# Animesh005/Torus-FHE

Measured on AMD Instinct MI355X. Metric: bootstrapped gates/sec (NAND, N=1024), higher is better.
Workload: dtype f64

## Files before the change

### torus-fhe_amd/csrc/thfhe_common.h

```cpp
#ifndef THFHE_COMMON_H
#define THFHE_COMMON_H

#include <hip/hip_runtime.h>

#include "../../include/thfhe_hip.h"
#include "thfhe_lane.h"

namespace thfhe {

constexpr int kOpIdentity = 100;

int thfhe_fail(int code, const char *msg);
int thfhe_fail_hip(hipError_t e, const char *what);

inline int ilog2(int x) {
    int l = 0;
    while ((1 << l) < x) l++;
    return l;
}

inline int lut_validate(const thfhe_lut_spec *sp, const void *tv, int n_luts, const int32_t *lut_index, const int32_t *in0, const int32_t *in1,
                        const int32_t *in2, const int32_t *out, size_t count, int max_luts = 1024) {
    if (!sp || !tv || !in0 || !out) return thfhe_fail(THFHE_E_INVALID, "null argument");
    if (sp->n_inputs < 1 || sp->n_inputs > 3) return thfhe_fail(THFHE_E_INVALID, "lut spec: n_inputs must be 1, 2 or 3");
// ... 76 lines not shown
    wave_sync();
    fwds_seg1(lane, z, xb, T1);
    wave_sync();
    fwds_seg2_ld(lane, z, xb);
    fwds_seg2_st(lane, z, xb, w);
    wave_sync();
    fwds_seg3(lane, z, xb);
}
__device__ __forceinline__ void wave_fft_inv_s(int lane, cplx (&z)[8], cplx *xb, const cplx *T1, const W64 &w) {
    wave_sync();
    invs_seg1(lane, z, xb, w);
    wave_sync();
    invs_seg2_ld(lane, z, xb);
    invs_seg2_st(lane, z, xb);
    wave_sync();
    invs_seg3(lane, z, xb, T1);
}
__device__ __forceinline__ void wave_fft_fwd_r(int lane, cplx (&z)[8], cplx *xb, const LaneRoots &r, const W64 &w) {
    wave_sync();
    fwdr_seg1(lane, z, xb, r);
    wave_sync();
    fwd_seg2_ld(lane, z, xb);
    fwdr_seg2_st(lane, z, xb, w);
    wave_sync();
    fwd_seg3(lane, z, xb);
}
__device__ __forceinline__ void wave_fft_inv_r(int lane, cplx (&z)[8], cplx *xb, const LaneRoots &r, const W64 &w) {
    wave_sync();
    invr_seg1(lane, z, xb, w);
    wave_sync();
    inv_seg2_ld(lane, z, xb);
    inv_seg2_st(lane, z, xb);
    wave_sync();
    invr_seg3(lane, z, xb, r);
}
__device__ __forceinline__ void wave_transpose_hi3(cplx (&z)[8]) {
    uint32_t w[8][4];
#pragma unroll
    for (int r = 0; r < 8; r++) __builtin_memcpy(w[r], &z[r], 16);
#pragma unroll
    for (int d = 0; d < 4; d++) {
#pragma unroll
        for (int r = 0; r < 4; r++) {
            auto q = __builtin_amdgcn_permlane32_swap(w[r][d], w[r + 4][d], false, false);
            w[r][d] = q[0];
            w[r + 4][d] = q[1];
        }
#pragma unroll
        for (int r = 0; r < 8; r++) {
            if (r & 2) continue;
            auto q = __builtin_amdgcn_permlane16_swap(w[r][d], w[r + 2][d], false, false);
            w[r][d] = q[0];
            w[r + 2][d] = q[1];
        }
#pragma unroll
        for (int r = 0; r < 8; r += 2) {
            const uint32_t a = w[r][d], b = w[r + 1][d];
            w[r + 1][d] = __builtin_amdgcn_update_dpp(b, a, 0x128, 0xF, 0x3, false);
            w[r][d] = __builtin_amdgcn_update_dpp(a, b, 0x128, 0xF, 0xC, false);
        }
    }
#pragma unroll
    for (int r = 0; r < 8; r++) __builtin_memcpy(&z[r], w[r], 16);
}
template <class Roots>
__device__ __forceinline__ void wave_fft_fwd_q(int lane, cplx (&z)[8], cplx *xb, const Roots &r, const W64 &w) {
    fwdq_seg1(z, r);
    wave_transpose_hi3(z);
    wave_sync();
    fwdr_seg2_st(lane, z, xb, w);
    wave_sync();
    fwd_seg3(lane, z, xb);
}
template <class Roots>
__device__ __forceinline__ void wave_fft_inv_q(int lane, cplx (&z)[8], cplx *xb, const Roots &r, const W64 &w) {
    wave_sync();
    invr_seg1(lane, z, xb, w);
    wave_sync();
    inv_seg2_ld(lane, z, xb);
    dft8<-1>(z);
    wave_transpose_hi3(z);
    invq_seg3(z, r);
}
template <class Roots>
__device__ __forceinline__ void wave_fft_fwd_qs(int lane, cplx (&z)[8], cplx *xb, const Roots &r, const W64 &w) {
    fwdq_seg1(z, r);
    wave_transpose_hi3(z);
    wave_sync();
    fwds_seg2_st(lane, z, xb, w);
    wave_sync();
    fwds_seg3(lane, z, xb);
}
template <class Roots>
__device__ __forceinline__ void wave_fft_inv_qs(int lane, cplx (&z)[8], cplx *xb, const Roots &r, const W64 &w) {
    wave_sync();
    invs_seg1(lane, z, xb, w);
    wave_sync();
    invs_seg2_ld(lane, z, xb);
    dft8<-1>(z);
    wave_transpose_hi3(z);
    invq_seg3(z, r);
}
template <int T>
__device__ __forceinline__ void wave_fft_fwd_t(int lane, cplx (&z)[8], cplx *xb, const cplx *T1t, const W64 &w) {
    wave_sync();
    fwdt_seg1<T>(lane, z, xb, T1t);
    wave_sync();
    fwds_seg2_ld(lane, z, xb);
    fwds_seg2_st(lane, z, xb, w);
    wave_sync();
    fwds_seg3(lane, z, xb);
}
template <int T>
__device__ __forceinline__ void wave_fft_inv_t(int lane, cplx (&z)[8], cplx *xb, const cplx *T1t, const W64 &w) {
    wave_sync();
    invs_seg1(lane, z, xb, w);
    wave_sync();
    invs_seg2_ld(lane, z, xb);
    invs_seg2_st(lane, z, xb);
    wave_sync();
    invt_seg3<T>(lane, z, xb, T1t);
}
template <int T, int DEN = 32>
__device__ __forceinline__ void wave_fft_fwd_tq(int lane, cplx (&z)[8], cplx *xb, const LaneRoots &r, const W64 &w) {
    fwdtq_seg1<T, DEN>(z, r);
    wave_transpose_hi3(z);
    wave_sync();
    fwds_seg2_st(lane, z, xb, w);
    wave_sync();
    fwds_seg3(lane, z, xb);
}
template <int T, int DEN = 32>
__device__ __forceinline__ void wave_fft_inv_tq(int lane, cplx (&z)[8], cplx *xb, const LaneRoots &r, const W64 &w) {
    wave_sync();
    invs_seg1(lane, z, xb, w);
    wave_sync();
    invs_seg2_ld(lane, z, xb);
    dft8<-1>(z);
    wave_transpose_hi3(z);
    invtq_seg3<T, DEN>(z, r);
}

template <int TA, int TB, int DEN = 32>
__device__ __forceinline__ void wave_fft_fwd_tq_two(int lane, cplx (&za)[8], cplx (&zb)[8], cplx *xa, cplx *xb, const LaneRoots &ra, const LaneRoots &rb,
                                                    const W64 &w) {
    fwdtq_seg1<TA, DEN>(za, ra);
    fwdtq_seg1<TB, DEN>(zb, rb);
    wave_transpose_hi3(za);
    wave_transpose_hi3(zb);
    wave_sync();
    fwds_seg2_st(lane, za, xa, w);
    fwds_seg2_st(lane, zb, xb, w);
    wave_sync();
    fwds_seg3(lane, za, xa);
    fwds_seg3(lane, zb, xb);
}
template <int TA, int TB, int DEN = 32>
__device__ __forceinline__ void wave_fft_inv_tq_two(int lane, cplx (&za)[8], cplx (&zb)[8], cplx *xb, const LaneRoots &ra, const LaneRoots &rb, const W64 &w) {
    wave_sync();
    invs_seg1(lane, za, xb, w);
    wave_sync();
    invs_seg2_ld(lane, za, xb);
    wave_sync();
    invs_seg1(lane, zb, xb, w);
    wave_sync();
    dft8<-1>(za);
// ... 13 lines not shown
```

### torus-fhe_amd/csrc/thfhe_lane.h

```cpp
#ifndef THFHE_LANE_H
#define THFHE_LANE_H

#include <limits.h>
#include <stddef.h>
#include <stdint.h>

#if defined(__HIPCC__)
#define THFHE_FN __host__ __device__ __forceinline__
#else
#define THFHE_FN inline __attribute__((always_inline))
#endif

namespace thfhe {

constexpr int kLanes = 64;
constexpr int kXbufSlots = 8 * 72;

struct alignas(16) cplx {
    double re, im;
};

THFHE_FN cplx cmul(cplx a, cplx b) { return cplx{a.re * b.re - a.im * b.im, a.re * b.im + a.im * b.re}; }
THFHE_FN cplx cmul_conj(cplx a, cplx b) {
    return cplx{a.re * b.re + a.im * b.im, a.im * b.re - a.re * b.im};
// ... 186 lines not shown
    dft8<+1>(z);
    cplx p[8];
    w64_powers(w, p);
    xbuf[xs_c(0, lane)] = z[0];
#pragma unroll
    for (int k1 = 1; k1 < 8; k1++) xbuf[xs_c(k1, lane)] = cmul(z[k1], p[k1]);
}
THFHE_FN void invr_seg1(int lane, cplx (&z)[8], cplx *xbuf, const W64 &w) {
    dft8<-1>(z);
    cplx p[8];
    w64_powers(w, p);
    xbuf[xs_d(0, lane)] = z[0];
#pragma unroll
    for (int j0 = 1; j0 < 8; j0++) xbuf[xs_d(j0, lane)] = cmul_conj(z[j0], p[j0]);
}
THFHE_FN void invr_seg3(int lane, cplx (&z)[8], const cplx *xbuf, const LaneRoots &r) {
    const cplx s2 = cmul(r.s, r.s);
    cplx e = r.b, o = cmul(r.b, r.s);
#pragma unroll
    for (int k0 = 0; k0 < 8; k0 += 2) {
        z[k0] = cmul_conj(xbuf[xs_a(k0, lane)], e);
        z[k0 + 1] = cmul_conj(xbuf[xs_a(k0 + 1, lane)], o);
        if (k0 < 6) {
            e = cmul(e, s2);
            o = cmul(o, s2);
        }
    }
    dft8<-1>(z);
#pragma unroll
    for (int m = 1; m < 8; m++) z[m] = cmul_conj(z[m], cplx{THFHE_C_RE(m), THFHE_C_IM(m)});
}

THFHE_FN void fwdq_seg1(cplx (&z)[8], const LaneRoots &r) {
#pragma unroll
    for (int m = 1; m < 8; m++) z[m] = cmul(z[m], cplx{THFHE_C_RE(m), THFHE_C_IM(m)});
    dft8<+1>(z);
    const cplx s2 = cmul(r.s, r.s);
    cplx e = r.b, o = cmul(r.b, r.s);
#pragma unroll
    for (int k0 = 0; k0 < 8; k0 += 2) {
        z[k0] = cmul(z[k0], e);
        z[k0 + 1] = cmul(z[k0 + 1], o);
        if (k0 < 6) {
            e = cmul(e, s2);
            o = cmul(o, s2);
        }
    }
}
THFHE_FN void invq_seg3(cplx (&z)[8], const LaneRoots &r) {
    const cplx s2 = cmul(r.s, r.s);
    cplx e = r.b, o = cmul(r.b, r.s);
#pragma unroll
    for (int k0 = 0; k0 < 8; k0 += 2) {
        z[k0] = cmul_conj(z[k0], e);
        z[k0 + 1] = cmul_conj(z[k0 + 1], o);
        if (k0 < 6) {
            e = cmul(e, s2);
            o = cmul(o, s2);
        }
    }
    dft8<-1>(z);
#pragma unroll
    for (int m = 1; m < 8; m++) z[m] = cmul_conj(z[m], cplx{THFHE_C_RE(m), THFHE_C_IM(m)});
}

struct LaneTw {
    cplx e[4], s;
};
THFHE_FN LaneTw make_lane_tw(const LaneRoots &r) {
    LaneTw t;
    const cplx s2 = cmul(r.s, r.s);
    t.e[0] = r.b;
#pragma unroll
    for (int j = 1; j < 4; j++) t.e[j] = cmul(t.e[j - 1], s2);
    t.s = r.s;
    return t;
}
THFHE_FN cplx opaque_cplx(cplx v) {
#if defined(__HIP_DEVICE_COMPILE__)
    asm volatile("" : "+v"(v.re), "+v"(v.im));
#endif
    return v;
}
THFHE_FN void fwdq_seg1(cplx (&z)[8], const LaneTw &t) {
#pragma unroll
    for (int m = 1; m < 8; m++) z[m] = cmul(z[m], cplx{THFHE_C_RE(m), THFHE_C_IM(m)});
    dft8<+1>(z);
    const cplx s = opaque_cplx(t.s);
#pragma unroll
    for (int j = 0; j < 4; j++) {
        z[2 * j] = cmul(z[2 * j], t.e[j]);
        z[2 * j + 1] = cmul(z[2 * j + 1], cmul(t.e[j], s));
    }
}
THFHE_FN void invq_seg3(cplx (&z)[8], const LaneTw &t) {
    const cplx s = opaque_cplx(t.s);
#pragma unroll
    for (int j = 0; j < 4; j++) {
        z[2 * j] = cmul_conj(z[2 * j], t.e[j]);
        z[2 * j + 1] = cmul_conj(z[2 * j + 1], cmul(t.e[j], s));
    }
    dft8<-1>(z);
#pragma unroll
    for (int m = 1; m < 8; m++) z[m] = cmul_conj(z[m], cplx{THFHE_C_RE(m), THFHE_C_IM(m)});
}

THFHE_FN uint32_t rot_minus_self32(const int32_t *p, int q, int a2n, int N) {
    int e = (q - a2n) & (2 * N - 1);
    uint32_t r = (uint32_t)p[e & (N - 1)];
    if (e & N) r = 0u - r;
    return r - (uint32_t)p[q];
}
THFHE_FN double digit32(uint32_t v, int shift, uint32_t mask, int32_t half) {
    return (double)((int32_t)((v >> shift) & mask) - half);
}
THFHE_FN uint32_t decomp_offset32(int l, int Bgbit) {
    uint32_t off = 0;
    for (int p = 1; p <= l; p++) off += (1u << (Bgbit - 1)) << (32 - p * Bgbit);
    return off;
}
THFHE_FN uint32_t round_lo32(double x) {
    double y = x + 6755399441055744.0;
    uint64_t b;
    __builtin_memcpy(&b, &y, 8);
    return (uint32_t)b;
}
THFHE_FN void split_limbs32(int32_t v, double &lo, double &hi) {
    int32_t l = (int32_t)(int16_t)(uint16_t)v;
    int32_t h = (int32_t)(((int64_t)v - l) >> 16);
    lo = (double)l;
    hi = (double)h;
}

THFHE_FN int32_t modswitch2n(int32_t x, int log2_2n) {
    int32_t y = (int32_t)((uint32_t)x + (1u << (32 - log2_2n - 1)));
    return y >> (32 - log2_2n);
}


THFHE_FN size_t bk_spec_index(int i, int r, int c, int h, int rows) {
    return ((((size_t)i * rows + r) * 2 + c) * 2 + h) * 512;
}

THFHE_FN void load_rotated16(int lane, const int32_t *acc_poly, int a2n, uint32_t offset, uint32_t (&t)[16]) {
    uint32_t r[16], s[16];
#pragma unroll
    for (int m = 0; m < 16; m++) {
        const int e = (lane + 64 * m - a2n) & 2047;
        r[m] = (uint32_t)acc_poly[e & 1023];
        s[m] = (uint32_t)acc_poly[lane + 64 * m];
    }
#if defined(__HIP_DEVICE_COMPILE__)
    __builtin_amdgcn_sched_barrier(0);
#endif
#pragma unroll
    for (int m = 0; m < 16; m++) {
        const int e = (lane + 64 * m - a2n) & 2047;
        t[m] = ((e & 1024) ? 0u - r[m] : r[m]) - s[m] + offset;
    }
}
THFHE_FN void digits_to_z(const uint32_t (&t)[16], int p, int Bgbit, cplx (&z)[8]) {
    const int shift = 32 - p * Bgbit;
    const uint32_t mask = (1u << Bgbit) - 1u;
    const int32_t half = 1 << (Bgbit - 1);
#pragma unroll
    for (int m = 0; m < 8; m++) z[m] = cplx{digit32(t[m], shift, mask, half), digit32(t[m + 8], shift, mask, half)};
}
THFHE_FN int32_t sbfe32(uint32_t v, int shift, int width) {
#if defined(__HIP_DEVICE_COMPILE__)
    return __builtin_amdgcn_sbfe((int32_t)v, (uint32_t)shift, (uint32_t)width);
#else
    return (int32_t)(v << (32 - shift - width)) >> (32 - width);
#endif
}
THFHE_FN void rotated_digits_z(int lane, const int32_t *p, int a2n, int level, int l, int Bgbit, cplx (&z)[8]) {
    const int shift = 32 - level * Bgbit;
    const uint32_t off = decomp_offset32(l, Bgbit) + ((1u << (Bgbit - 1)) << shift);
    const uint32_t e4 = ((uint32_t)(lane - a2n) & 2047u) << 2;
#if defined(__HIP_DEVICE_COMPILE__)
    const uint32_t base = (uint32_t)(size_t)(__attribute__((address_space(3))) const void *)p;
#endif
    uint32_t r[8][2], s[8][2];
#pragma unroll
    for (int m = 0; m < 8; m++) {
#pragma unroll
        for (int q = 0; q < 2; q++) {
            const int c = lane + 64 * m + 512 * q;
// ... 416 lines not shown
    constexpr double C8 = 0.923879532511286756128, S8 = 0.382683432365089771728, R = 0.70710678118654752440;
    z[1] = cplx{z[1].re * C8 - z[1].im * S8, z[1].re * S8 + z[1].im * C8};
    z[2] = cplx{(z[2].re - z[2].im) * R, (z[2].re + z[2].im) * R};
    z[3] = cplx{z[3].re * S8 - z[3].im * C8, z[3].re * C8 + z[3].im * S8};
}
template <int QT>
THFHE_FN cplx comb4096(const cplx (&u)[4]) {
    if (QT == 0) return cplx{u[0].re + u[1].re + u[2].re + u[3].re, u[0].im + u[1].im + u[2].im + u[3].im};
    if (QT == 1) return cplx{u[0].re - u[1].im - u[2].re + u[3].im, u[0].im + u[1].re - u[2].im - u[3].re};
    if (QT == 2) return cplx{u[0].re - u[1].re + u[2].re - u[3].re, u[0].im - u[1].im + u[2].im - u[3].im};
    return cplx{u[0].re + u[1].im - u[2].re - u[3].im, u[0].im - u[1].re - u[2].im + u[3].re};
}
THFHE_FN void merge4096(const cplx &a0, const cplx &a1, const cplx &a2, const cplx &a3, cplx (&z)[4]) {
    constexpr double C8 = 0.923879532511286756128, S8 = 0.382683432365089771728, R = 0.70710678118654752440;
    z[0] = cplx{a0.re + a1.re + a2.re + a3.re, a0.im + a1.im + a2.im + a3.im};
    const cplx v1{a0.re + a1.im - a2.re - a3.im, a0.im - a1.re - a2.im + a3.re};
    const cplx v2{a0.re - a1.re + a2.re - a3.re, a0.im - a1.im + a2.im - a3.im};
    const cplx v3{a0.re - a1.im - a2.re + a3.im, a0.im + a1.re - a2.im - a3.re};
    z[1] = cplx{v1.re * C8 + v1.im * S8, v1.im * C8 - v1.re * S8};
    z[2] = cplx{(v2.re + v2.im) * R, (v2.im - v2.re) * R};
    z[3] = cplx{v3.re * S8 + v3.im * C8, v3.im * S8 - v3.re * C8};
}
template <int NN>
THFHE_FN uint64_t rot_minus_self64_n(const int64_t *p, int q, int a2n) {
    int e = (q - a2n) & (2 * NN - 1);
    uint64_t r = (uint64_t)p[e & (NN - 1)];
    if (e & NN) r = 0ull - r;
    return r - (uint64_t)p[q];
}
template <int NN, int K>
THFHE_FN void rot_minus_self64_batch(const int64_t *p, int q0, int a2n, uint64_t (&out)[K]) {
    uint64_t r[K], s[K];
#pragma unroll
    for (int k = 0; k < K; k++) {
        const int e = (q0 + 64 * k - a2n) & (2 * NN - 1);
        r[k] = (uint64_t)p[e & (NN - 1)];
        s[k] = (uint64_t)p[q0 + 64 * k];
    }
#if defined(__HIP_DEVICE_COMPILE__)
    __builtin_amdgcn_sched_barrier(0);
#endif
#pragma unroll
    for (int k = 0; k < K; k++) {
        const int e = (q0 + 64 * k - a2n) & (2 * NN - 1);
        out[k] = ((e & NN) ? 0ull - r[k] : r[k]) - s[k];
    }
}
THFHE_FN void load_rotated32_hi(int lane, const int64_t *acc_poly, int a2n, uint64_t offset, uint32_t (&t)[32]) {
#pragma unroll
    for (int m = 0; m < 32; m++) t[m] = (uint32_t)((rot_minus_self64_n<2048>(acc_poly, lane + 64 * m, a2n) + offset) >> 32);
}
THFHE_FN void digits_to_z16(const uint32_t (&t)[32], int p, int Bgbit, cplx (&z)[16]) {
    const int shift = 32 - p * Bgbit;
    const uint32_t mask = (1u << Bgbit) - 1u;
    const int32_t half = 1 << (Bgbit - 1);
#pragma unroll
    for (int m = 0; m < 16; m++) z[m] = cplx{digit32(t[m], shift, mask, half), digit32(t[m + 16], shift, mask, half)};
}
template <int NN>
THFHE_FN void acc_init_64_n(int lane, int64_t *acc_mask, int64_t *acc_body, int barb, int64_t mu) {
#pragma unroll
    for (int m = 0; m < NN / 64; m++) {
        int q = lane + 64 * m;
        int e = (q + barb) & (2 * NN - 1);
        acc_mask[q] = 0;
        acc_body[q] = (e & NN) ? (int64_t)(0ull - (uint64_t)mu) : mu;
    }
}
template <int NN>
THFHE_FN void extract_64_n(int lane, const int64_t *acc_mask, const int64_t *acc_body, int32_t *out) {
#pragma unroll
    for (int m = 0; m < NN / 64; m++) {
        int q = lane + 64 * m;
        out[q] = t64tot32(q == 0 ? acc_mask[0] : (int64_t)(0ull - (uint64_t)acc_mask[NN - q]));
    }
    if (lane == 0) out[NN] = t64tot32(acc_body[0]);
}
THFHE_FN size_t mk_chunk_index_2k(long pi, int r, int h, int o, int rows) { return mk_chunk_index(pi, r, h, o, rows) * 2; }

struct TwRing1k {
    static constexpr int T1 = 0;
    static constexpr int T2 = 512;
    static constexpr int ROOTS = 576;
    static constexpr int SIZE = 704;
};
struct TwRing2k {
    static constexpr int T1_TWIST1 = 0;
    static constexpr int T1_TWIST5 = 512;
    static constexpr int T2 = 1024;
    static constexpr int RATIO = 1088;
    static constexpr int ROOTS4K = 1152;
    static constexpr int SIZE = 1408;
};
template <int NN>
THFHE_FN constexpr int tw_t2() { return NN == 1024 ? TwRing1k::T2 : TwRing2k::T2; }

}

#include <cmath>
#include <vector>
#pragma GCC visibility push(hidden)
namespace thfhe {
inline void make_twiddles_t2(cplx *T2 ) {
    const long double PI = 3.14159265358979323846264338327950288L;
    for (int k1 = 0; k1 < 8; k1++)
        for (int j0 = 0; j0 < 8; j0++) {
            long double ang = 2.0L * PI * (long double)(j0 * k1) / 64.0L;
            T2[k1 * 8 + j0] = cplx{(double)cosl(ang), (double)sinl(ang)};
        }
}
inline void make_twiddles_1024(cplx *T1 , cplx *T2 ) {
    const long double PI = 3.14159265358979323846264338327950288L;
    for (int k0 = 0; k0 < 8; k0++)
        for (int lane = 0; lane < 64; lane++) {
            long double ang = PI * (long double)(lane * (4 * k0 + 1)) / 1024.0L;
            T1[k0 * 64 + lane] = cplx{(double)cosl(ang), (double)sinl(ang)};
        }
    make_twiddles_t2(T2);
}
inline void make_lane_roots_1024(cplx *roots ) {
    const long double PI = 3.14159265358979323846264338327950288L;
    for (int lane = 0; lane < 64; lane++) {
        long double a = PI * (long double)lane / 1024.0L, b = PI * (long double)(4 * lane) / 1024.0L;
        roots[2 * lane] = cplx{(double)cosl(a), (double)sinl(a)};
        roots[2 * lane + 1] = cplx{(double)cosl(b), (double)sinl(b)};
    }
}
inline void make_lane_ratio_2048(cplx *s ) {
    const long double PI = 3.14159265358979323846264338327950288L;
    for (int lane = 0; lane < 64; lane++) {
        long double a = PI * (long double)(8 * lane) / 2048.0L;
        s[lane] = cplx{(double)cosl(a), (double)sinl(a)};
    }
}
inline void make_lane_roots_4096(cplx *roots ) {
    const long double PI = 3.14159265358979323846264338327950288L;
    for (int q = 0; q < 4; q++)
        for (int lane = 0; lane < 64; lane++) {
            long double a = PI * (long double)((4 * q + 1) * lane) / 4096.0L;
            roots[q * 64 + lane] = cplx{(double)cosl(a), (double)sinl(a)};
        }
}
inline void make_twiddles_2048(cplx *T1a , cplx *T1b ) {
    const long double PI = 3.14159265358979323846264338327950288L;
    for (int k0 = 0; k0 < 8; k0++)
        for (int lane = 0; lane < 64; lane++) {
            long double a1 = PI * (long double)(lane * (8 * k0 + 1)) / 2048.0L, a5 = PI * (long double)(lane * (8 * k0 + 5)) / 2048.0L;
            T1a[k0 * 64 + lane] = cplx{(double)cosl(a1), (double)sinl(a1)};
            T1b[k0 * 64 + lane] = cplx{(double)cosl(a5), (double)sinl(a5)};
        }
}
inline std::vector<cplx> make_twiddle_table(int N) {
    if (N == 1024) {
        std::vector<cplx> tw(TwRing1k::SIZE);
        make_twiddles_1024(tw.data() + TwRing1k::T1, tw.data() + TwRing1k::T2);
        make_lane_roots_1024(tw.data() + TwRing1k::ROOTS);
        return tw;
    }
    std::vector<cplx> tw(TwRing2k::SIZE);
    make_twiddles_2048(tw.data() + TwRing2k::T1_TWIST1, tw.data() + TwRing2k::T1_TWIST5);
    make_twiddles_t2(tw.data() + TwRing2k::T2);
    make_lane_ratio_2048(tw.data() + TwRing2k::RATIO);
    make_lane_roots_4096(tw.data() + TwRing2k::ROOTS4K);
    return tw;
}
}
#pragma GCC visibility pop

#endif
```

### torus-fhe_amd/csrc/thfhe_sk.hip

```cpp
#include <hip/hip_runtime.h>

#include <algorithm>
#include <cstdlib>
#include <memory>
#include <mutex>
#include <new>
#include <string>
#include <vector>

#include "../../include/thfhe_hip.h"
#include "thfhe_common.h"
#include "thfhe_dag.h"
#include "thfhe_devctx.h"
#include "thfhe_keyswitch.h"
#include "thfhe_lane.h"
#include "thfhe_pack.h"

using namespace thfhe;

namespace {

#include "thfhe_transform.h"

struct Lin {
    int32_t cb, cx, cy;
    int ysel;
};
__host__ __device__ inline bool gate_lin(int op, int which, Lin &L) {
    const int32_t E8 = 1 << 29, E4 = 1 << 30;
    switch (op) {
    case THFHE_NAND: L = Lin{E8, -1, -1, 1}; return true;
    case THFHE_OR: L = Lin{E8, 1, 1, 1}; return true;
    case THFHE_AND: L = Lin{-E8, 1, 1, 1}; return true;
    case THFHE_XOR: L = Lin{E4, 2, 2, 1}; return true;
    case THFHE_XNOR: L = Lin{-E4, -2, -2, 1}; return true;
    case THFHE_NOR: L = Lin{-E8, -1, -1, 1}; return true;
    case THFHE_ANDNY: L = Lin{-E8, -1, 1, 1}; return true;
    case THFHE_ANDYN: L = Lin{-E8, 1, -1, 1}; return true;
    case THFHE_ORNY: L = Lin{E8, -1, 1, 1}; return true;
    case THFHE_ORYN: L = Lin{E8, 1, -1, 1}; return true;
    case THFHE_MUX: L = which == 0 ? Lin{-E8, 1, 1, 1} : Lin{-E8, -1, 1, 2}; return true;
    case kOpIdentity: L = Lin{0, 1, 0, 1}; return true;
    default: return false;
    }
}

__global__ __launch_bounds__(256) void sk_prologue_kernel(const int32_t *__restrict__ in0, const int32_t *__restrict__ in1,
                                                           const int32_t *__restrict__ in2, int op, const int32_t *__restrict__ ops,
                                                           int rot_per_gate, int n, int n_pad, int log2_2n, long jobs,
                                                           int32_t *__restrict__ bara, int32_t *__restrict__ barb) {
    const long job = blockIdx.y;
    const int i = blockIdx.x * 256 + threadIdx.x;
    if (job >= jobs || i > n) return;
    const long gate = job / rot_per_gate;
    const int which = (int)(job % rot_per_gate);
    Lin L;
    gate_lin(ops ? ops[gate] : op, which, L);
    const size_t off = (size_t)gate * (n + 1) + i;
    uint32_t v = (uint32_t)L.cx * (uint32_t)in0[off];
    if (L.cy != 0) v += (uint32_t)L.cy * (uint32_t)(L.ysel == 2 ? in2[off] : in1[off]);
    if (i == n) {
        v += (uint32_t)L.cb;
        barb[job] = modswitch2n((int32_t)v, log2_2n);
    } else {
        bara[job * n_pad + i] = modswitch2n((int32_t)v, log2_2n);
    }
}

THFHE_STAMP_STORAGE

struct BRArgs {
    const cplx *bk;
    const cplx *tw;
    const int32_t *bara;
    const int32_t *barb;
    int32_t *out;
    long jobs;
    int n, n_pad, Bgbit;
    int32_t mu;
    const int32_t *tv;
    const int32_t *lut_idx;
    int theta;
    const int32_t *tv_a;
    const int32_t *mv_w;
    int mv_p, mv_box;
};

constexpr int kGate = 0, kLut = 1, kLutEnc = 2, kLutMv = 3;

#ifndef THFHE_RING_NF
#define THFHE_RING_NF 16
#endif
#ifndef THFHE_RING_LEAN_ROOTS
#define THFHE_RING_LEAN_ROOTS 1
#endif
#ifndef THFHE_RING_READ_FIRST
#define THFHE_RING_READ_FIRST 0
#endif
template <int L, int V = 1, int W = 8, int LUT = kGate>
__global__ __launch_bounds__(64 * W, W == 8 ? 2 : 1) void sk_blind_rotate_ring_kernel(BRArgs a) {
    __shared__ __attribute__((aligned(4096))) int32_t sAcc[W][2048];
    __shared__ cplx sX[W][kXbufSlots];
    __shared__ cplx sRing[3][512];
    constexpr int ROWS = 2 * L;
    constexpr int DPC = 8 / W;
    const int wave = __builtin_amdgcn_readfirstlane(threadIdx.x >> 6);
    const int lane = threadIdx.x & 63;
    const W64 w64{a.tw[TwRing1k::T2 + 1 * 8 + (lane & 7)]};
    const LaneRoots roots{a.tw[TwRing1k::ROOTS + 2 * lane], a.tw[TwRing1k::ROOTS + 2 * lane + 1]};
    const LaneTw tw = make_lane_tw(roots);
    const long job = (long)blockIdx.x * W + wave;
    const bool has_job = job < a.jobs;
    int32_t *acc = sAcc[wave];
    cplx *xb = sX[wave];
    const uniform_i32_ptr bara = as_uniform(a.bara + (has_job ? job : 0) * a.n_pad);
    const int Bgbit = a.Bgbit;
    if (has_job) {
        if constexpr (LUT == kLutEnc) {
            const size_t t = a.lut_idx ? (size_t)a.lut_idx[job] * 1024 : 0;
            acc_init_tlwe16(lane, acc, acc + 1024, a.barb[job], a.tv_a + t, a.tv + t);
        } else if constexpr (LUT == kLutMv) acc_init_tv16(lane, acc, acc + 1024, a.barb[job], a.tv);
        else if constexpr (LUT) acc_init_tv16(lane, acc, acc + 1024, a.barb[job], a.tv + (a.lut_idx ? (size_t)a.lut_idx[job] * 1024 : 0));
        else acc_init16(lane, acc, acc + 1024, a.barb[job], a.mu);
    }

    const long total_chunks = (long)a.n * ROWS * 4;
    const cplx *gsrc = a.bk + wave * (64 * DPC) + lane;
    long q_issue = 0;
    int slot_issue = 0;
    const uint32_t ring_base = (uint32_t)(size_t)(__attribute__((address_space(3))) void *)&sRing[0][0] + (uint32_t)wave * (1024u * DPC);
    auto issue = [&]() {
#pragma unroll
        for (int d = 0; d < DPC; d++) ring_dma(gsrc + 64 * d, ring_base + (uint32_t)slot_issue * 8192u + 1024u * d);
        if (q_issue + 1 < total_chunks) {
            gsrc += 512;
            q_issue++;
        }
        slot_issue = slot_issue == 2 ? 0 : slot_issue + 1;
    };
    __syncthreads();
    issue();
    issue();
    issue();
    int slot_use = 0;
    STAMP_DECL;

    for (int i = 0; i < a.n; i++) {
        const int ai = bara[i];
        const bool active = has_job && ai != 0;
        const int a2n = ai & 2047;
        cplx S[2][2][8];
#pragma unroll
        for (int c = 0; c < 2; c++)
#pragma unroll
            for (int h = 0; h < 2; h++)
#pragma unroll
                for (int m = 0; m < 8; m++) S[c][h][m] = cplx{0.0, 0.0};
        constexpr int NF = THFHE_RING_NF;
        uint32_t fld[NF];
#pragma unroll
        for (int r = 0; r < ROWS; r++) {
            cplx z[8];
            if (active) {
                int a2n_r = a2n;
                asm volatile("" : "+s"(a2n_r));
                if (r % L == 0) rotated_fields_keep<NF, W == 4>(lane, acc + (r / L) * 1024, a2n_r, L, Bgbit, fld);
                asm volatile("" : "+s"(a2n_r));
                mixed_digits_z<NF>(lane, acc + (r / L) * 1024, a2n_r, (r % L) + 1, L, Bgbit, fld, z);
                if (!(V & 1)) wave_fft_fwd_r(lane, z, xb, roots, w64);
                else if (THFHE_RING_LEAN_ROOTS && W == 8) wave_fft_fwd_q(lane, z, xb, LaneRoots{opaque_cplx(roots.b), opaque_cplx(roots.s)}, w64);
                else wave_fft_fwd_q(lane, z, xb, tw, w64);
            }
            STAMP(0);
            cplx bA[4], bB[4];
#pragma unroll
            for (int c4 = 0; c4 < 4; c4++) {
                if (c4 == 0) ring_barrier<2 * DPC>(); else ring_barrier<DPC>();
                STAMP(1);
                const cplx *B = &sRing[slot_use][0];
#if THFHE_RING_READ_FIRST
                if (active) {
#pragma unroll
                    for (int m = 0; m < 4; m++) bA[m] = B[m * 64 + lane];
                }
                __builtin_amdgcn_sched_barrier(0);
                if (c4 > 0) issue();
                if (active) {
#else
                if (c4 > 0) issue();
                if (active) {
#pragma unroll
                    for (int m = 0; m < 4; m++) bA[m] = B[m * 64 + lane];
#endif
                    if (c4 > 0) {
#pragma unroll
                        for (int m = 0; m < 4; m++) cfma(S[(c4 - 1) >> 1][(c4 - 1) & 1][4 + m], z[4 + m], bB[m]);
                    }
#pragma unroll
                    for (int m = 0; m < 4; m++) bB[m] = B[(4 + m) * 64 + lane];
#pragma unroll
                    for (int m = 0; m < 4; m++) cfma(S[c4 >> 1][c4 & 1][m], z[m], bA[m]);
                }
                slot_use = slot_use == 2 ? 0 : slot_use + 1;
                STAMP(2);
            }
            ring_barrier<2 * DPC>();
            issue();
            STAMP(1);
            if (active) {
#pragma unroll
                for (int m = 0; m < 4; m++) cfma(S[1][1][4 + m], z[4 + m], bB[m]);
            }
            STAMP(2);
        }
        if (active) {
            wave_sync();
#pragma unroll
            for (int c = 0; c < 2; c++) {
                if ((V & 1) && !(V & 2)) {
                    if (THFHE_RING_LEAN_ROOTS && W == 8) {
                        wave_fft_inv_q(lane, S[c][0], xb, LaneRoots{opaque_cplx(roots.b), opaque_cplx(roots.s)}, w64);
                        wave_fft_inv_q(lane, S[c][1], xb, LaneRoots{opaque_cplx(roots.b), opaque_cplx(roots.s)}, w64);
                    } else {
                        wave_fft_inv_q(lane, S[c][0], xb, tw, w64);
                        wave_fft_inv_q(lane, S[c][1], xb, tw, w64);
                    }
                } else {
                    wave_fft_inv_r(lane, S[c][0], xb, roots, w64);
                    wave_fft_inv_r(lane, S[c][1], xb, roots, w64);
                }
                acc_update16(lane, acc + c * 1024, S[c][0], S[c][1]);
            }
            wave_sync();
        }
        STAMP(3);
    }
    STAMP_FLUSH(blockIdx.x, wave);
    asm volatile("s_waitcnt vmcnt(0)" ::: "memory");
    if (has_job) {
        if constexpr (LUT == kLutMv) {
            const uniform_i32_ptr w = as_uniform(a.mv_w) + (size_t)(a.lut_idx ? as_uniform(a.lut_idx)[job] : 0) * a.theta * a.mv_p;
            for (int j = 0; j < a.theta; j++) extract_mv16(lane, acc, acc + 1024, w + j * a.mv_p, a.mv_p, a.mv_box, a.out + (job * a.theta + j) * 1025);
        } else if constexpr (LUT) {
            for (int j = 0; j < a.theta; j++) extract_at16(lane, acc, acc + 1024, j, a.out + (job * a.theta + j) * 1025);
        } else {
            extract16(lane, acc, acc + 1024, a.out + job * 1025);
        }
    }
}

__device__ __forceinline__ void wg_barrier() { asm volatile("s_waitcnt lgkmcnt(0)\n\ts_barrier" ::: "memory"); }
__device__ __forceinline__ void pin() { asm volatile("" ::: "memory"); }

template <int L, int PACE = 1, int LUT = kGate>
__global__ __launch_bounds__(512, 2) void sk_blind_rotate_coop_kernel(BRArgs a) {
    constexpr int ROWS = 2 * L;
    __shared__ __attribute__((aligned(4096))) int32_t sAcc[2048];
    __shared__ cplx sSpec[ROWS][512];
    __shared__ cplx sX[8][kXbufSlots];
    const int wave = __builtin_amdgcn_readfirstlane(threadIdx.x >> 6);
    const int lane = threadIdx.x & 63;
    const W64 w64{a.tw[TwRing1k::T2 + 1 * 8 + (lane & 7)]};
    const LaneRoots roots{a.tw[TwRing1k::ROOTS + 2 * lane], a.tw[TwRing1k::ROOTS + 2 * lane + 1]};
    const long job = blockIdx.x;
    const uniform_i32_ptr bara = as_uniform(a.bara + job * a.n_pad);
    const int Bgbit = a.Bgbit;
    if (wave == 0) {
        if constexpr (LUT == kLutEnc) {
            const size_t t = a.lut_idx ? (size_t)a.lut_idx[job] * 1024 : 0;
            acc_init_tlwe16(lane, sAcc, sAcc + 1024, a.barb[job], a.tv_a + t, a.tv + t);
        } else if constexpr (LUT == kLutMv) acc_init_tv16(lane, sAcc, sAcc + 1024, a.barb[job], a.tv);
        else if constexpr (LUT) acc_init_tv16(lane, sAcc, sAcc + 1024, a.barb[job], a.tv + (a.lut_idx ? (size_t)a.lut_idx[job] * 1024 : 0));
        else acc_init16(lane, sAcc, sAcc + 1024, a.barb[job], a.mu);
    }
    const int c = (wave >> 1) & 1, h = wave & 1, half = wave >> 2, r0 = half * L;
    unsigned int *ap = reinterpret_cast<unsigned int *>(sAcc) + c * 1024;
    cplx *xb = sX[wave];

    int i = 0;
    while (i < a.n && bara[i] == 0) i++;
    cplx B[L][8];
    if (i < a.n) {
#pragma unroll
        for (int r = 0; r < L; r++) load8(lane, B[r], a.bk + bk_spec_index(i, r0 + r, c, h, ROWS));
    }
    wg_barrier();
    STAMP_DECL;
    while (i < a.n) {
        const int a2n = bara[i] & 2047;
        int inext = i + 1;
        while (inext < a.n && bara[inext] == 0) inext++;
        const int inl = inext < a.n ? inext : i;
        if (wave < ROWS) {
            cplx z[8];
            rotated_digits_z(lane, sAcc + (wave / L) * 1024, a2n, (wave % L) + 1, L, Bgbit, z);
            wave_fft_fwd_q(lane, z, xb, roots, w64);
#pragma unroll
            for (int m = 0; m < 8; m++) sSpec[wave][m * 64 + lane] = z[m];
        }
        STAMP(0);
        wg_barrier();
        STAMP(1);
// ... 66 lines not shown
        i = inext;
    }
    STAMP_FLUSH(blockIdx.x, wave);
    if constexpr (LUT == kLutMv) {
        const uniform_i32_ptr w = as_uniform(a.mv_w) + (size_t)(a.lut_idx ? as_uniform(a.lut_idx)[job] : 0) * a.theta * a.mv_p;
        for (int j = wave; j < a.theta; j += 8)
            extract_mv16(lane, sAcc, sAcc + 1024, w + j * a.mv_p, a.mv_p, a.mv_box, a.out + (job * a.theta + j) * 1025);
    } else if constexpr (LUT) {
        if (wave < a.theta) extract_at16(lane, sAcc, sAcc + 1024, wave, a.out + (job * a.theta + wave) * 1025);
    } else {
        if (wave == 0) extract16(lane, sAcc, sAcc + 1024, a.out + job * 1025);
    }
}

__global__ __launch_bounds__(256) void sk_linear_kernel(const int32_t *__restrict__ in0, int32_t *__restrict__ out, size_t words, int negate) {
    const size_t q = (size_t)blockIdx.x * 256 + threadIdx.x;
    if (q < words) out[q] = negate ? (int32_t)(0u - (uint32_t)in0[q]) : in0[q];
}

}

struct THFHE_INTERNAL thfhe_ctx : DevCtx {
    thfhe_params p;
    DevBuf d_bk;
    KsKey ksk;
    int coop_max_jobs = 768;
    int ring4_max_jobs = 1024;
    int n_pad = 0;
    DevBuf d_bara, d_barb, d_u;
    DevBuf d_tv, d_lut_idx;
    DevBuf d_tva;
    DevBuf d_mv_w;
    DevBuf d_tree_tab, d_tree_lwe, d_tree_a, d_tree_b;
    DevBuf d_dag_enc_a, d_dag_enc_b, d_dag_tv1;
    DevBuf d_dag_mv_tv0, d_dag_mv_w;
    DevBuf d_dag_lhe_tab_a, d_dag_lhe_tab_b, d_dag_lhe_fin_a, d_dag_lhe_fin_b, d_dag_lhe_words;
    DevBuf d_lhe_a, d_lhe_b, d_lhe_in[4];
    DevBuf d_wfa_tab;
    DevBuf d_sc_tab, d_sc_idx;
    int cus = 0;
    int wfa_chunk = 0;
    size_t tree_slice = 65536;
    Stage stage;
    DagBuffers dag;
    size_t dag_slice = 28672;
    hipEvent_t grp_ev[2] = {nullptr, nullptr};
    bool grp_valid = false;
    ~thfhe_ctx() {
        for (hipEvent_t e : grp_ev)
            if (e) (void)hipEventDestroy(e);
    }
};

struct THFHE_INTERNAL thfhe_tgsw_set {
    thfhe_ctx *ctx = nullptr;
    DevBuf spec;
    size_t count = 0;
    int d = 0;
};

namespace {

constexpr int kMaxEncLuts = 1 << 18;

int ensure_workspace(thfhe_ctx *c, size_t jobs) {
    int rc = c->d_bara.grow(jobs * c->n_pad * sizeof(int32_t));
    if (!rc) rc = c->d_barb.grow(jobs * sizeof(int32_t));
    if (!rc) rc = c->d_u.grow(jobs * 1025 * sizeof(int32_t));
    return rc;
}

template <int L, int LUT>
void launch_coop(const BRArgs &a, hipStream_t s) {
#ifdef THFHE_VARIANTS
    static const int pace = std::getenv("THFHE_COOP_PACE") ? std::atoi(std::getenv("THFHE_COOP_PACE")) : 1;
    if (!LUT && pace == 0) { hipLaunchKernelGGL((sk_blind_rotate_coop_kernel<L, 0>), dim3((unsigned)a.jobs), dim3(512), 0, s, a); return; }
    if (!LUT && pace == 2) { hipLaunchKernelGGL((sk_blind_rotate_coop_kernel<L, 2>), dim3((unsigned)a.jobs), dim3(512), 0, s, a); return; }
    if (!LUT && pace == 4) { hipLaunchKernelGGL((sk_blind_rotate_coop_kernel<L, 4>), dim3((unsigned)a.jobs), dim3(512), 0, s, a); return; }
#endif
    hipLaunchKernelGGL((sk_blind_rotate_coop_kernel<L, 1, LUT>), dim3((unsigned)a.jobs), dim3(512), 0, s, a);
}
template <int L, int LUT>
void launch_ring4(const BRArgs &a, hipStream_t s) {
    hipLaunchKernelGGL((sk_blind_rotate_ring_kernel<L, 1, 4, LUT>), dim3((unsigned)((a.jobs + 3) / 4)), dim3(256), 0, s, a);
}
template <int L, int LUT>
void launch_ring8(const BRArgs &a, hipStream_t s) {
    const dim3 grid((unsigned)((a.jobs + 7) / 8)), block(512);
#ifdef THFHE_VARIANTS
    static const int variant = std::getenv("THFHE_RING_VARIANT") ? std::atoi(std::getenv("THFHE_RING_VARIANT")) : 0;
    if (!LUT && variant == 8) { hipLaunchKernelGGL((sk_blind_rotate_ring_kernel<L, 0>), grid, block, 0, s, a); return; }
    if (!LUT && variant == 3) { hipLaunchKernelGGL((sk_blind_rotate_ring_kernel<L, 3>), grid, block, 0, s, a); return; }
#endif
    hipLaunchKernelGGL((sk_blind_rotate_ring_kernel<L, 1, 8, LUT>), grid, block, 0, s, a);
}

template <int L, int LUT>
void launch_br(const BRArgs &a, hipStream_t s, int coop_max, int ring4_max) {
    auto piece = [&](long first, long count) {
        BRArgs b = a;
        b.bara += first * a.n_pad, b.barb += first, b.jobs = count;
        b.out += first * (LUT ? a.theta : 1) * 1025;
        if (LUT && b.lut_idx) b.lut_idx += first;
        return b;
    };
    constexpr long kRound = 2048;
    const long full = (coop_max > 0 || ring4_max > 0) ? a.jobs / kRound * kRound : a.jobs;
    if (full > 0) launch_ring8<L, LUT>(piece(0, full), s);
    const long r = a.jobs - full;
    if (r == 0) return;
    if (r <= coop_max) launch_coop<L, LUT>(piece(full, r), s);
    else if (r <= ring4_max) launch_ring4<L, LUT>(piece(full, r), s);
    else if (ring4_max > 0 && coop_max > 0 && r <= ring4_max + (coop_max < 256 ? coop_max : 256)) {
        launch_ring4<L, LUT>(piece(full, ring4_max), s);
        launch_coop<L, LUT>(piece(full + ring4_max, r - ring4_max), s);
    } else launch_ring8<L, LUT>(piece(full, r), s);
}

template <int LUT>
int launch_rotations(thfhe_ctx *c, const BRArgs &a) {
    switch (c->p.l) {
    case 1: launch_br<1, LUT>(a, c->stream, c->coop_max_jobs, c->ring4_max_jobs); break;
    case 2: launch_br<2, LUT>(a, c->stream, c->coop_max_jobs, c->ring4_max_jobs); break;
    case 3: launch_br<3, LUT>(a, c->stream, c->coop_max_jobs, c->ring4_max_jobs); break;
    case 4: launch_br<4, LUT>(a, c->stream, c->coop_max_jobs, c->ring4_max_jobs); break;
    default: return thfhe_fail(THFHE_E_UNSUPPORTED, "decomposition length l must be 1..4");
    }
    return THFHE_OK;
}

int enqueue_rotations(thfhe_ctx *c, int op, const int32_t *d0, const int32_t *d1, const int32_t *d2, size_t gates,
                      int rot_per_gate, int32_t mu, const int32_t *d_ops = nullptr) {
    const size_t jobs = gates * rot_per_gate;
    int rc = ensure_workspace(c, jobs);
    if (rc) return rc;
    const int n = c->p.n;
    if (c->profiling) THFHE_HIP(hipEventRecord(c->ev[0], c->stream));
    dim3 pg((unsigned)((n + 1 + 255) / 256), (unsigned)jobs);
    hipLaunchKernelGGL(sk_prologue_kernel, pg, dim3(256), 0, c->stream, d0, d1, d2, op, d_ops, rot_per_gate, n, c->n_pad,
                       ilog2(2 * c->p.N), (long)jobs, c->d_bara.as<int32_t>(), c->d_barb.as<int32_t>());
    if (c->profiling) THFHE_HIP(hipEventRecord(c->ev[1], c->stream));
    BRArgs a{c->d_bk.as<cplx>(), c->d_tw.as<cplx>(), c->d_bara.as<int32_t>(), c->d_barb.as<int32_t>(), c->d_u.as<int32_t>(), (long)jobs, n, c->n_pad, c->p.Bgbit, mu};
    rc = launch_rotations<kGate>(c, a);
    if (rc) return rc;
    if (c->profiling) THFHE_HIP(hipEventRecord(c->ev[2], c->stream));
    THFHE_HIP(hipGetLastError());
    return THFHE_OK;
}

int enqueue_keyswitch(thfhe_ctx *c, const int32_t *d_u, int32_t *d_out, size_t gates, int rot_per_gate, bool timed) {
    KsArgs k = c->ksk.args(d_u, d_out, (long)gates);
    k.rot_per_gate = rot_per_gate;
    const int nsplit = gates <= 32 ? 16 : (gates <= 128 ? 8 : (gates <= 512 ? 2 : 1));
    THFHE_TRY(ks_enqueue(c->ksk, k, nsplit, c->stream));
    if (timed && c->profiling) {
        THFHE_HIP(hipEventRecord(c->ev[3], c->stream));
        c->ev_valid = true;
    }
    return THFHE_OK;
}

struct MvArgs {
    const int32_t *w;
    int p;
};

template <typename Src>
int enqueue_pbs(thfhe_ctx *c, const Src &src, size_t jobs, const int32_t *tv, const int32_t *tv_a, int theta, const int32_t *d_idx, int32_t *ks_dst,
                bool timed = false, const MvArgs *mv = nullptr) {
    const int n = c->p.n;
    const bool ev = timed && c->profiling;
    int32_t *const idx = c->d_lut_idx.as<int32_t>();
    if (ev) THFHE_HIP(hipEventRecord(c->ev[0], c->stream));
    lut_prologue_launch(src, jobs, n, c->n_pad, ilog2(2 * c->p.N), c->d_bara.as<int32_t>(), c->d_barb.as<int32_t>(), idx, c->stream);
    if (ev) THFHE_HIP(hipEventRecord(c->ev[1], c->stream));
    BRArgs a{c->d_bk.as<cplx>(), c->d_tw.as<cplx>(), c->d_bara.as<int32_t>(), c->d_barb.as<int32_t>(), c->d_u.as<int32_t>(), (long)jobs, n, c->n_pad, c->p.Bgbit,
             0, tv, Src::kIdx == LutIdx::none ? d_idx : idx, theta, tv_a};
// ... 764 lines not shown
```

Before: 135,600.

## Fold FFT twists into twiddled radix-8 butterflies with FMA-based kernels

Adds a new FFT variant (V&4) for the N=1024 ring blind-rotate kernel. It merges the per-lane twist multiplies into radix-8 stages built from twiddled butterflies that use FMAs, driven by a new per-lane roots table. It becomes the default for the ring8 and ring4 launches. The aim is fewer FP64 complex multiplies and less register pressure in the forward and inverse FFTs, at the cost of recomputing root powers per call and some possible numerical drift.

```diff
diff --git a/torus-fhe_amd/csrc/thfhe_common.h b/torus-fhe_amd/csrc/thfhe_common.h
--- a/torus-fhe_amd/csrc/thfhe_common.h
+++ b/torus-fhe_amd/csrc/thfhe_common.h
@@ -182,6 +182,25 @@
     wave_transpose_hi3(z);
     invq_seg3(z, r);
 }
+__device__ __forceinline__ void wave_fft_fwd_f(int lane, cplx (&z)[8], cplx *xb, const LaneRootsF &r) {
+    fwdf_seg1(z);
+    wave_transpose_hi3(z);
+    wave_sync();
+    fwdf_seg2_st(lane, z, xb, r);
+    wave_sync();
+    fwdf_seg3(lane, z, xb, r);
+}
+template <bool LEAN>
+__device__ __forceinline__ void wave_fft_inv_f(int lane, cplx (&z)[8], cplx *xb, W64 &w, LaneRoots &r, const cplx (&bc)[4]) {
+    if (LEAN) opaque_in_place(w.w1), opaque_in_place(r.s);
+    wave_sync();
+    invf_seg1(lane, z, xb);
+    wave_sync();
+    inv_seg2_ld(lane, z, xb);
+    invf_seg2(z, w);
+    wave_transpose_hi3(z);
+    invf_seg3(z, r, bc);
+}
 template <class Roots>
 __device__ __forceinline__ void wave_fft_fwd_qs(int lane, cplx (&z)[8], cplx *xb, const Roots &r, const W64 &w) {
     fwdq_seg1(z, r);
diff --git a/torus-fhe_amd/csrc/thfhe_lane.h b/torus-fhe_amd/csrc/thfhe_lane.h
--- a/torus-fhe_amd/csrc/thfhe_lane.h
+++ b/torus-fhe_amd/csrc/thfhe_lane.h
@@ -292,6 +292,11 @@
 #endif
     return v;
 }
+THFHE_FN void opaque_in_place(cplx &v) {
+#if defined(__HIP_DEVICE_COMPILE__)
+    asm volatile("" : "+v"(v.re), "+v"(v.im));
+#endif
+}
 THFHE_FN void fwdq_seg1(cplx (&z)[8], const LaneTw &t) {
 #pragma unroll
     for (int m = 1; m < 8; m++) z[m] = cmul(z[m], cplx{THFHE_C_RE(m), THFHE_C_IM(m)});
@@ -313,6 +318,95 @@
     dft8<-1>(z);
 #pragma unroll
     for (int m = 1; m < 8; m++) z[m] = cmul_conj(z[m], cplx{THFHE_C_RE(m), THFHE_C_IM(m)});
+}
+
+THFHE_FN void bfly_tw(cplx &a, cplx &b, cplx W) {
+    const cplx x{__builtin_fma(-W.im, b.im, __builtin_fma(W.re, b.re, a.re)), __builtin_fma(W.im, b.re, __builtin_fma(W.re, b.im, a.im))};
+    b = cplx{__builtin_fma(2.0, a.re, -x.re), __builtin_fma(2.0, a.im, -x.im)};
+    a = x;
+}
+THFHE_FN void bfly_c4(cplx &a, cplx &b) {
+    constexpr double R = 0.70710678118654752440;
+    const double t = b.re - b.im, u = b.re + b.im;
+    b = cplx{__builtin_fma(-R, t, a.re), __builtin_fma(-R, u, a.im)};
+    a = cplx{__builtin_fma(R, t, a.re), __builtin_fma(R, u, a.im)};
+}
+struct RootPow {
+    cplx w1, w2, w4, w1o;
+};
+THFHE_FN cplx csqr(cplx a) { return cplx{__builtin_fma(a.re, a.re, -(a.im * a.im)), (a.re + a.re) * a.im}; }
+template <int S>
+THFHE_FN RootPow root_powers(cplx w) {
+    constexpr double R = 0.70710678118654752440;
+    RootPow p;
+    p.w1 = w;
+    p.w2 = csqr(w);
+    p.w4 = csqr(p.w2);
+    p.w1o = S > 0 ? cplx{R * (w.re - w.im), R * (w.re + w.im)} : cplx{R * (w.re + w.im), R * (w.im - w.re)};
+    return p;
+}
+template <int S>
+THFHE_FN void dft8_tw_tail(cplx (&y)[8], cplx w1, cplx w2, cplx w1o) {
+    bfly_tw(y[0], y[2], w2);
+    bfly_tw(y[1], y[3], w2);
+    bfly_tw(y[4], y[6], mul_si<S>(w2));
+    bfly_tw(y[5], y[7], mul_si<S>(w2));
+    bfly_tw(y[0], y[1], w1);
+    bfly_tw(y[2], y[3], mul_si<S>(w1));
+    bfly_tw(y[4], y[5], w1o);
+    bfly_tw(y[6], y[7], mul_si<S>(w1o));
+    const cplx x4 = y[1], x2 = y[2], x6 = y[3], x1 = y[4], x5 = y[5], x3 = y[6];
+    y[1] = x1;
+    y[2] = x2;
+    y[3] = x3;
+    y[4] = x4;
+    y[5] = x5;
+    y[6] = x6;
+}
+template <int S>
+THFHE_FN void dft8_tw(cplx (&y)[8], const RootPow &p) {
+#pragma unroll
+    for (int m = 0; m < 4; m++) bfly_tw(y[m], y[m + 4], p.w4);
+    dft8_tw_tail<S>(y, p.w1, p.w2, p.w1o);
+}
+THFHE_FN void dft8_tw_c32(cplx (&y)[8]) {
+#pragma unroll
+    for (int m = 0; m < 4; m++) bfly_c4(y[m], y[m + 4]);
+    dft8_tw_tail<+1>(y, cplx{THFHE_C_RE(1), THFHE_C_IM(1)}, cplx{THFHE_C_RE(2), THFHE_C_IM(2)}, cplx{THFHE_C_RE(5), THFHE_C_IM(5)});
+}
+struct LaneRootsF {
+    cplx s, w;
+};
+THFHE_FN void fwdf_seg1(cplx (&z)[8]) { dft8_tw_c32(z); }
+THFHE_FN void fwdf_seg2_st(int lane, cplx (&z)[8], cplx *xbuf, const LaneRootsF &r) {
+    dft8_tw<+1>(z, root_powers<+1>(r.s));
+#pragma unroll
+    for (int k1 = 0; k1 < 8; k1++) xbuf[xs_c(k1, lane)] = z[k1];
+}
+THFHE_FN void fwdf_seg3(int lane, cplx (&z)[8], const cplx *xbuf, const LaneRootsF &r) {
+    fwd_seg3_ld(lane, z, xbuf);
+    dft8_tw<+1>(z, root_powers<+1>(r.w));
+}
+THFHE_FN cplx cconj(cplx a) { return cplx{a.re, -a.im}; }
+THFHE_FN void make_untwist_f(cplx b, cplx (&bc)[4]) {
+    bc[0] = b;
+#pragma unroll
+    for (int m = 1; m < 4; m++) bc[m] = cmul(b, cplx{THFHE_C_RE(m), THFHE_C_IM(m)});
+}
+THFHE_FN void invf_seg1(int lane, cplx (&z)[8], cplx *xbuf) {
+    dft8<-1>(z);
+#pragma unroll
+    for (int j0 = 0; j0 < 8; j0++) xbuf[xs_d(j0, lane)] = z[j0];
+}
+THFHE_FN void invf_seg2(cplx (&z)[8], const W64 &w) { dft8_tw<-1>(z, root_powers<-1>(cconj(w.w1))); }
+THFHE_FN void invf_seg3(cplx (&z)[8], const LaneRoots &r, const cplx (&bc)[4]) {
+    constexpr double R = 0.70710678118654752440;
+    dft8_tw<-1>(z, root_powers<-1>(cconj(r.s)));
+#pragma unroll
+    for (int m = 0; m < 4; m++) {
+        z[m] = cmul_conj(z[m], bc[m]);
+        z[m + 4] = cmul_conj(cplx{R * (z[m + 4].re + z[m + 4].im), R * (z[m + 4].im - z[m + 4].re)}, bc[m]);
+    }
 }
 
 THFHE_FN uint32_t rot_minus_self32(const int32_t *p, int q, int a2n, int N) {
@@ -895,7 +989,8 @@
     static constexpr int T1 = 0;
     static constexpr int T2 = 512;
     static constexpr int ROOTS = 576;
-    static constexpr int SIZE = 704;
+    static constexpr int ROOTSF = 704;
+    static constexpr int SIZE = 832;
 };
 struct TwRing2k {
     static constexpr int T1_TWIST1 = 0;
@@ -939,6 +1034,15 @@
         roots[2 * lane + 1] = cplx{(double)cosl(b), (double)sinl(b)};
     }
 }
+inline void make_lane_roots_f_1024(cplx *roots ) {
+    const long double PI = 3.14159265358979323846264338327950288L;
+    for (int lane = 0; lane < 64; lane++) {
+        const int k0 = lane >> 3, k1 = lane & 7;
+        long double a = PI * (long double)(8 * (4 * k0 + 1)) / 1024.0L, b = PI * (long double)(32 * k1 + 4 * k0 + 1) / 1024.0L;
+        roots[2 * lane] = cplx{(double)cosl(a), (double)sinl(a)};
+        roots[2 * lane + 1] = cplx{(double)cosl(b), (double)sinl(b)};
+    }
+}
 inline void make_lane_ratio_2048(cplx *s ) {
     const long double PI = 3.14159265358979323846264338327950288L;
     for (int lane = 0; lane < 64; lane++) {
@@ -968,6 +1072,7 @@
         std::vector<cplx> tw(TwRing1k::SIZE);
         make_twiddles_1024(tw.data() + TwRing1k::T1, tw.data() + TwRing1k::T2);
         make_lane_roots_1024(tw.data() + TwRing1k::ROOTS);
+        make_lane_roots_f_1024(tw.data() + TwRing1k::ROOTSF);
         return tw;
     }
     std::vector<cplx> tw(TwRing2k::SIZE);
diff --git a/torus-fhe_amd/csrc/thfhe_sk.hip b/torus-fhe_amd/csrc/thfhe_sk.hip
--- a/torus-fhe_amd/csrc/thfhe_sk.hip
+++ b/torus-fhe_amd/csrc/thfhe_sk.hip
@@ -97,7 +97,7 @@
 #ifndef THFHE_RING_READ_FIRST
 #define THFHE_RING_READ_FIRST 0
 #endif
-template <int L, int V = 1, int W = 8, int LUT = kGate>
+template <int L, int V = 5, int W = 8, int LUT = kGate>
 __global__ __launch_bounds__(64 * W, W == 8 ? 2 : 1) void sk_blind_rotate_ring_kernel(BRArgs a) {
     __shared__ __attribute__((aligned(4096))) int32_t sAcc[W][2048];
     __shared__ cplx sX[W][kXbufSlots];
@@ -109,6 +109,9 @@
     const W64 w64{a.tw[TwRing1k::T2 + 1 * 8 + (lane & 7)]};
     const LaneRoots roots{a.tw[TwRing1k::ROOTS + 2 * lane], a.tw[TwRing1k::ROOTS + 2 * lane + 1]};
     const LaneTw tw = make_lane_tw(roots);
+    LaneRootsF rootsf{a.tw[TwRing1k::ROOTSF + 2 * lane], a.tw[TwRing1k::ROOTSF + 2 * lane + 1]};
+    W64 w64f = w64;
+    LaneRoots rootsi = roots;
     const long job = (long)blockIdx.x * W + wave;
     const bool has_job = job < a.jobs;
     int32_t *acc = sAcc[wave];
@@ -167,7 +170,10 @@
                 if (r % L == 0) rotated_fields_keep<NF, W == 4>(lane, acc + (r / L) * 1024, a2n_r, L, Bgbit, fld);
                 asm volatile("" : "+s"(a2n_r));
                 mixed_digits_z<NF>(lane, acc + (r / L) * 1024, a2n_r, (r % L) + 1, L, Bgbit, fld, z);
-                if (!(V & 1)) wave_fft_fwd_r(lane, z, xb, roots, w64);
+                if (V & 4) {
+                    if (THFHE_RING_LEAN_ROOTS && W == 8) opaque_in_place(rootsf.s), opaque_in_place(rootsf.w);
+                    wave_fft_fwd_f(lane, z, xb, rootsf);
+                } else if (!(V & 1)) wave_fft_fwd_r(lane, z, xb, roots, w64);
                 else if (THFHE_RING_LEAN_ROOTS && W == 8) wave_fft_fwd_q(lane, z, xb, LaneRoots{opaque_cplx(roots.b), opaque_cplx(roots.s)}, w64);
                 else wave_fft_fwd_q(lane, z, xb, tw, w64);
             }
@@ -215,9 +221,17 @@
         }
         if (active) {
             wave_sync();
+            cplx bc[4];
+            if (V & 4) {
+                if (THFHE_RING_LEAN_ROOTS && W == 8) opaque_in_place(rootsi.b);
+                make_untwist_f(rootsi.b, bc);
+            }
 #pragma unroll
             for (int c = 0; c < 2; c++) {
-                if ((V & 1) && !(V & 2)) {
+                if (V & 4) {
+                    wave_fft_inv_f<THFHE_RING_LEAN_ROOTS && W == 8>(lane, S[c][0], xb, w64f, rootsi, bc);
+                    wave_fft_inv_f<THFHE_RING_LEAN_ROOTS && W == 8>(lane, S[c][1], xb, w64f, rootsi, bc);
+                } else if ((V & 1) && !(V & 2)) {
                     if (THFHE_RING_LEAN_ROOTS && W == 8) {
                         wave_fft_inv_q(lane, S[c][0], xb, LaneRoots{opaque_cplx(roots.b), opaque_cplx(roots.s)}, w64);
                         wave_fft_inv_q(lane, S[c][1], xb, LaneRoots{opaque_cplx(roots.b), opaque_cplx(roots.s)}, w64);
@@ -450,7 +464,7 @@
 }
 template <int L, int LUT>
 void launch_ring4(const BRArgs &a, hipStream_t s) {
-    hipLaunchKernelGGL((sk_blind_rotate_ring_kernel<L, 1, 4, LUT>), dim3((unsigned)((a.jobs + 3) / 4)), dim3(256), 0, s, a);
+    hipLaunchKernelGGL((sk_blind_rotate_ring_kernel<L, 5, 4, LUT>), dim3((unsigned)((a.jobs + 3) / 4)), dim3(256), 0, s, a);
 }
 template <int L, int LUT>
 void launch_ring8(const BRArgs &a, hipStream_t s) {
@@ -458,9 +472,10 @@
 #ifdef THFHE_VARIANTS
     static const int variant = std::getenv("THFHE_RING_VARIANT") ? std::atoi(std::getenv("THFHE_RING_VARIANT")) : 0;
     if (!LUT && variant == 8) { hipLaunchKernelGGL((sk_blind_rotate_ring_kernel<L, 0>), grid, block, 0, s, a); return; }
+    if (!LUT && variant == 1) { hipLaunchKernelGGL((sk_blind_rotate_ring_kernel<L, 1>), grid, block, 0, s, a); return; }
     if (!LUT && variant == 3) { hipLaunchKernelGGL((sk_blind_rotate_ring_kernel<L, 3>), grid, block, 0, s, a); return; }
 #endif
-    hipLaunchKernelGGL((sk_blind_rotate_ring_kernel<L, 1, 8, LUT>), grid, block, 0, s, a);
+    hipLaunchKernelGGL((sk_blind_rotate_ring_kernel<L, 5, 8, LUT>), grid, block, 0, s, a);
 }
 
 template <int L, int LUT>
```

Measured after the change: 139,800, median of 6. 3.1% higher.
